# rmcolq/charon

Measured on AMD Instinct MI355X. Metric: classified reads/sec + achieved HBM GB/s vs roofline, 5 kb reads, 39 GB index, higher is better.
Workload: dtype u64

## Files before the change

charon_amd/csrc/charon_hip.hip:

```cpp

#include <hip/hip_runtime.h>

#include <algorithm>
#include <chrono>
#include <functional>
#include <cmath>
#include <cstddef>
#include <cstdint>
#include <cstdio>
#include <cstdlib>
#include <cstring>
#include <limits>
#include <mutex>
#include <new>
#include <string>
#include <type_traits>
#include <vector>

#include "charon_hip.h"
#include "default_kde.inc"

#include "parts/common.inc"
#include "parts/lds_budget.hpp"
#include "parts/k1_minimise_probe.inc"
#include "parts/k2_count_wavelog.inc"
#include "parts/shard_kernels.inc"
#include "parts/shardx_kernels.inc"
#include "parts/k3_model_call.inc"
#include "parts/len_order.inc"
#include "parts/gzip_trees.inc"
#include "parts/gzip_walk.inc"
#include "parts/gzip_tally.inc"
#include "parts/gzip_size_dev.inc"
#include "parts/gzip_tally_long.inc"
#include "parts/text_pack.inc"
#include "parts/text_split.inc"
#include "parts/fasta_split.inc"
#include "parts/text_gather.inc"
#include "parts/text_pair.inc"
#include "parts/extract_records.inc"
#include "parts/inflate_members.inc"
#include "parts/deflate_members.inc"
#include "parts/ef_decode.inc"
#include "parts/synth_kernels.inc"
#include "parts/abi_index_model.inc"
#include "parts/abi_stream_batch.inc"
#include "parts/abi_shard_wait.inc"
#include "parts/abi_text_split.inc"
#include "parts/abi_fasta_split.inc"
#include "parts/abi_text_fetch.inc"
#include "parts/abi_text_pair.inc"
#include "parts/abi_text_batch.inc"
#include "parts/abi_inflate.inc"
#include "parts/abi_deflate.inc"
#include "parts/abi_extract.inc"
#include "parts/abi_shardx.inc"
#include "parts/abi_synth_memory.inc"
```

charon_amd/csrc/parts/abi_shard_wait.inc:

```

static int ensure_shard_buffers(chn_stream *s) {
    const uint64_t nw = (s->cfg.max_reads + WAVE - 1) / WAVE;
    int rc;
    if ((rc = s->big.ensure(s->cfg.max_bases, nw, (uint32_t)s->idx->d.bin_words, 65536, 0))) return rc;
    if ((rc = s->d_list.ensure(s->big.log_cap * 8)) || (rc = s->d_cbase.ensure((nw + 1) * 8))) return rc;
    return CHN_OK;
}
static ShardArgs shard_args(chn_stream *s, const chn_index *shard, uint64_t *partial, const Slot &sl) {
    ShardArgs a;
    std::memset(&a, 0, sizeof a);
    const chn_index_desc &d = shard->d;
    a.list = s->d_list.as<uint64_t>(); a.wave_meta = s->big.meta.as<WaveMeta>(); a.cbase = s->d_cbase.as<uint64_t>();
    a.wave_count = s->big.wcount.as<uint32_t>(); a.words = shard->words; a.S = d.bin_size; a.row_begin = d.row_begin; a.row_end = d.row_end;
    a.shift = (uint32_t)d.hash_shift; a.h = d.hash_funs; a.W = (uint32_t)d.bin_words; a.partial = partial; a.rows = s->big.rows.as<uint64_t>();
    a.rowlog = s->big.log.as<uint32_t>(); a.B = (uint32_t)d.bins;
    a.n_waves = (uint32_t)((sl.n_reads + WAVE - 1) / WAVE); a.esc_capacity = s->big.esc_cap;
    a.status = reinterpret_cast<uint32_t *>(const_cast<Slot &>(sl).d_ctl.as<unsigned long long>() + CTL_STATUS);
    return a;
}

extern "C" int chn_shard_minimise(chn_stream *s, const chn_batch *b, uint64_t *n_entries) {
    if (!s || !b || !n_entries) return fail(CHN_E_INVALID, "chn_shard_minimise: null argument");
    if (s->shard_open || s->shx_stage != 0) return fail(CHN_E_STATE, "chn_shard_minimise: previous sharded batch not finished");
    HIPCHK(hipSetDevice(s->idx->d.device));
// ... 84 lines not shown
    HIPCHK(hipStreamSynchronize(s->stream));
    return CHN_OK;
}

extern "C" int chn_shard_finish(chn_stream *s, const uint64_t *dev_partial) {
    if (!s) return fail(CHN_E_INVALID, "chn_shard_finish: null argument");
    if (!s->shard_open) return fail(CHN_E_STATE, "chn_shard_finish: no sharded batch open");
    if (!dev_partial && s->shard_entries) return fail(CHN_E_INVALID, "chn_shard_finish: null argument");
    HIPCHK(hipSetDevice(s->idx->d.device));
    Slot &sl = s->slot[s->head];
    const uint32_t n_waves = (uint32_t)((sl.n_reads + WAVE - 1) / WAVE);
    const ShardArgs sa = shard_args(s, s->idx, const_cast<uint64_t *>(dev_partial), sl);
    switch (s->idx->d.bin_words) {
        case 1: hipLaunchKernelGGL(k_and_partial<1>, dim3(n_waves), dim3(256), 0, s->stream, sa); break;
        case 2: hipLaunchKernelGGL(k_and_partial<2>, dim3(n_waves), dim3(256), 0, s->stream, sa); break;
        case 3: hipLaunchKernelGGL(k_and_partial<3>, dim3(n_waves), dim3(256), 0, s->stream, sa); break;
        default: hipLaunchKernelGGL(k_and_partial<4>, dim3(n_waves), dim3(256), 0, s->stream, sa); break;
    }
    HIPCHK(hipGetLastError());
    s->shard_open = false;
    HIPCHK(hipEventRecord(sl.k1_done, s->stream));
    HIPCHK(hipStreamWaitEvent(s->stream2, sl.k1_done, 0));
    int rc = launch_tail(s, sl, s->big, s->stream2);
    if (rc) return rc;
    s->head = (s->head + 1) % chn_stream::N_SLOTS;
    s->inflight += 1;
    return CHN_OK;
}

extern "C" int chn_stream_sync(chn_stream *s) {
    if (!s) return fail(CHN_E_INVALID, "null stream");
    HIPCHK(hipSetDevice(s->idx->d.device));
    HIPCHK(hipStreamSynchronize(s->stream0));
    HIPCHK(hipStreamSynchronize(s->stream));
    HIPCHK(hipStreamSynchronize(s->stream1));
    HIPCHK(hipStreamSynchronize(s->stream4));
    HIPCHK(hipStreamSynchronize(s->stream2));
    return CHN_OK;
}

static int rerun_worst_case(chn_stream *s, Slot &sl) {
    const chn_index_desc &d = s->idx->d;
    unsigned long long *ctl = sl.d_ctl.as<unsigned long long>();
    const uint64_t n = sl.n_reads, nw = (n + WAVE - 1) / WAVE + sl.split_bound;
    HIPCHK(hipMemsetAsync(ctl, 0, CTL_NLONG * 8, s->stream));
    HIPCHK(hipMemsetAsync(ctl + CTL_FETCHES, 0, (CTL_WORDS - CTL_FETCHES) * 8, s->stream));
    hipLaunchKernelGGL(k_sum_len, dim3((uint32_t)std::min<uint64_t>(1024, (n + 255) / 256)), dim3(256), 0, s->stream, sl.len1, sl.len2, (uint32_t)n, ctl + CTL_WORDS - 1);
    HIPCHK(hipGetLastError());
    unsigned long long total = 0;
    HIPCHK(hipMemcpyAsync(&total, ctl + CTL_WORDS - 1, 8, hipMemcpyDeviceToHost, s->stream));
    HIPCHK(hipStreamSynchronize(s->stream));
    int rc = s->big.ensure(total, (n + WAVE - 1) / WAVE + std::min<uint64_t>(sl.split_bound, total / len_bucket_floor(std::min(s->long_bucket, 247u)) + 1), (uint32_t)d.bin_words, 65536, 0, nw);
    if (rc) return rc;
    K1Args a = sl.k1;
    a.gate_started = a.gate_signal = nullptr;
    fill_k1_log(a, sl, s->big, true);
    const size_t lds = k1_lds_bytes(a.wn, d.num_categories, MODE_ROWS, a.h, (uint32_t)d.bin_words, (uint32_t)d.bins, a.pack != 0);
    hipError_t e = launch_k1_mode(MODE_ROWS, (uint32_t)d.bin_words, a, lds, s->stream);
    if (e == hipSuccess && sl.split_bound) e = launch_k1_split_mode(MODE_ROWS, (uint32_t)d.bin_words, a, lds, s->stream, split_grid(sl.split_bound));
    if (e != hipSuccess) return fail(CHN_E_HIP, std::string("k_minimise_probe re-run: ") + hipGetErrorString(e));
    if ((rc = launch_tail(s, sl, s->big, s->stream))) return rc;
    HIPCHK(hipStreamSynchronize(s->stream));
    s->overflow_reruns += 1;
    return CHN_OK;
}

extern "C" int chn_batch_wait(chn_stream *s, chn_result *r) {
    if (!s || !r || r->struct_size != sizeof(chn_result)) return fail(CHN_E_INVALID, "chn_batch_wait: bad argument");
    if (s->inflight == 0) return fail(CHN_E_STATE, "no batch in flight");
    HIPCHK(hipSetDevice(s->idx->d.device));
    Slot &sl = s->slot[(s->head + chn_stream::N_SLOTS - s->inflight) % chn_stream::N_SLOTS];
    static const bool diag_wait = diag_env("CHN_DIAG_WAIT") != nullptr;
    auto dnow = []() { return std::chrono::duration<double>(std::chrono::steady_clock::now().time_since_epoch()).count(); };
    const double dw0 = diag_wait ? dnow() : 0;
    HIPCHK(hipEventSynchronize(sl.done));
    const double dw1 = diag_wait ? dnow() : 0;
    if (sl.want_gzt) HIPCHK(hipEventSynchronize(sl.gz_done));
    const double dw2 = diag_wait ? dnow() : 0;
    struct DiagPrint { bool on; double a, b, c; std::function<double()> now; ~DiagPrint() { if (on) std::fprintf(stderr, "chn_batch_wait: at %.4f  done-event %.2f ms  gz-event %.2f ms  rest %.2f ms\n", a, (b - a) * 1e3, (c - b) * 1e3, (now() - c) * 1e3); } } diag_print{diag_wait, dw0, dw1, dw2, dnow};
    s->inflight -= 1;
    static const int evpair[4][2] = {{0, 1}, {2, 3}, {4, 5}, {6, 7}};
    for (int i = 0; i < 4; ++i)
        if (sl.ev_used[i]) {
            float ms = 0;
            HIPCHK(hipEventElapsedTime(&ms, sl.ev[evpair[i][0]], sl.ev[evpair[i][1]]));
            if (i == 0) {
                float t0 = 0, t1 = 0;
                HIPCHK(hipEventElapsedTime(&t0, s->prof_anchor[s->prof_cur], sl.ev[0]));
                HIPCHK(hipEventElapsedTime(&t1, s->prof_anchor[s->prof_cur], sl.ev[1]));
                if (s->prof_have_end && s->prof_prev_end > (double)t0) ms = (float)std::max(0.0, (double)t1 - s->prof_prev_end);
                if (!s->prof_have_end || (double)t1 > s->prof_prev_end) s->prof_prev_end = t1;
                s->prof_have_end = true;
                if (sl.new_anchor) {
                    float off = 0;
                    HIPCHK(hipEventElapsedTime(&off, s->prof_anchor[s->prof_cur], s->prof_anchor[s->prof_cur ^ 1]));
                    s->prof_prev_end -= off; s->prof_cur ^= 1;
                    sl.new_anchor = s->prof_anchor_pending = false;
                }
            }
            s->prof_ms[i] += ms; s->prof_n[i] += 1;
        }
    unsigned long long ctl[CTL_WORDS];
    const uint64_t n = sl.n_reads, C = s->idx->d.num_categories;
    const ResLayout L(n, C);
    const char *staged = sl.staged ? sl.h_res.as<char>() : nullptr;
    if (staged) std::memcpy(ctl, staged + L.ctl, sizeof ctl);
// ... 193 lines not shown
```

charon_amd/csrc/parts/abi_stream_batch.inc:

```

struct ResLayout {
    size_t ctl, prob, nh, counts, unique, call, conf, flags, total;
    ResLayout(uint64_t n, uint64_t C) {
        ctl = 0; prob = CTL_WORDS * 8; nh = prob + n * C * 8; counts = nh + n * 4; unique = counts + n * C * 4; call = unique + n * C * 4;
        conf = call + n; flags = conf + n; total = flags + n;
    }
};

static const int PROF_ANCHOR_SECONDS = 8;
static hipError_t prof_anchor_now(chn_stream *s) {
    for (Slot &sl : s->slot) sl.new_anchor = false;
    s->prof_cur = 0; s->prof_anchor_pending = false; s->prof_have_end = false; s->prof_prev_end = 0;
    hipError_t e = hipEventRecord(s->prof_anchor[0], s->stream);
    if (e == hipSuccess) e = hipEventSynchronize(s->prof_anchor[0]);
    s->prof_anchor_at = std::chrono::steady_clock::now();
    return e;
}

extern "C" int chn_stream_create(chn_index *idx, const chn_stream_cfg *cfg, chn_stream **out) {
    if (!idx || !cfg || !out || cfg->struct_size != sizeof(chn_stream_cfg)) return fail(CHN_E_INVALID, "chn_stream_create: bad argument");
    if (cfg->max_reads == 0 || cfg->max_reads > 0xFFFFFF00ULL) return fail(CHN_E_INVALID, "max_reads out of range");
    HIPCHK(hipSetDevice(idx->d.device));
    idx->ef_release();
    chn_stream *s = new (std::nothrow) chn_stream();
// ... 516 lines not shown
    HIPCHK(hipGetLastError());
    HIPCHK(hipEventRecord(sl.uploaded, s->stream0));
    HIPCHK(hipStreamWaitEvent(ps, sl.uploaded, 0));

    K1Args &a = sl.k1;
    std::memset(&a, 0, sizeof(a));
    a.words = s->idx->words; a.S = d.bin_size; a.row_begin = d.row_begin; a.row_end = d.row_end; a.seed = d.minimiser_seed; a.powk1 = pow5(d.kmer_size - 1);
    a.shift = (uint32_t)d.hash_shift; a.h = d.hash_funs; a.k = d.kmer_size; a.wn = d.window_size - d.kmer_size + 1;
    a.n_reads = (uint32_t)n; a.nseg = paired ? 2 : 1; a.B = (uint32_t)d.bins; a.C = C;
    a.pack = ring_pack_ok(a.k, a.wn, a.seed) ? 1u : 0u;
    for (uint32_t bb = 0; bb < 8 && bb < d.bins; ++bb) a.b2c_packed |= (uint64_t)d.bin_to_category[bb] << (8 * bb);
    a.bases = bases; a.nmask = nmask; a.off1 = off1; a.off2 = off2; a.len1 = sl.len1; a.len2 = sl.len2; a.n_bases = b->n_bases;
    a.order = sl.d_order.as<uint32_t>();
    a.status = reinterpret_cast<uint32_t *>(ctl + CTL_STATUS);
    if (const char *ab = diag_env("CHN_ABLATE")) a.ablate = (uint32_t)std::atoi(ab);
    a.nt_probes = s->idx->rows_local * d.bin_words * 8 > (4ULL << 30) ? 1u : 0u;
    if (const char *nt = diag_env("CHN_NT_PROBES")) a.nt_probes = (uint32_t)std::atoi(nt);
    a.num_hashes = sl.d_num_hashes.as<uint32_t>(); a.counts = sl.d_counts.as<uint32_t>(); a.unique = sl.d_unique.as<uint32_t>();
    const uint32_t n_waves = (uint32_t)((n + WAVE - 1) / WAVE);
    a.n_long_ptr = sl.split_bound ? ctl + CTL_NLONG : nullptr; a.wave_slot0 = n_waves;
    a.fetches = ctl + CTL_FETCHES;
    if (list_kind == LIST_SPARSE) {
        fill_k1_log(a, sl, s->shx, true);
        a.rows = s->d_list.as<uint64_t>();
    } else if (list_mode) {
        fill_k1_log(a, sl, s->big, false);
        a.rows = s->d_list.as<uint64_t>();
        hipLaunchKernelGGL(k_wave_caps, dim3((uint32_t)((n + 255) / 256)), dim3(256), 0, ps, sl.d_order.as<uint32_t>(), sl.len1, sl.len2,
                           (uint32_t)n, s->big.cap_num, s->big.esc_shift, s->big.meta.as<WaveMeta>());
        hipLaunchKernelGGL(k_scan_meta, dim3(1), dim3(1024), 0, ps, s->big.meta.as<WaveMeta>(), n_waves);
        HIPCHK(hipGetLastError());
    } else if (!fused) {
        fill_k1_log(a, sl, sl.lb, true);
    }
    const int mode = list_mode ? MODE_LIST : fused ? MODE_FUSED : MODE_ROWS;
    size_t lds = k1_lds_bytes(a.wn, C, mode, a.h, W, a.B, a.pack != 0);
    if (const char *pad = diag_env("CHN_LDS_PAD")) lds += (size_t)std::atoi(pad);
    if (lds > 160 * 1024) return fail(CHN_E_INVALID, "window too large for LDS");
    if (sl.split_bound) {
        HIPCHK(hipStreamWaitEvent(s->stream4, sl.uploaded, 0));
        hipError_t e4 = launch_k1_split_mode(mode, W, a, lds, s->stream4, split_grid(sl.split_bound));
        if (e4 != hipSuccess) return fail(CHN_E_HIP, std::string("k_minimise_probe (split) launch: ") + hipGetErrorString(e4));
        HIPCHK(hipEventRecord(sl.split_done, s->stream4));
    }
    const bool gated = !list_mode && alternate && s->gate_signal != nullptr;
    if (gated) {
        if (s->gate_seq) {
            HIPCHK(hipStreamWaitValue64(ps, s->gate_signal, s->gate_seq, hipStreamWaitValueGte, ~0ull));
            s->gated_batches += 1;
        }
        a.gate_started = ctl + CTL_GATE; a.gate_signal = s->gate_signal; a.gate_value = s->gate_seq + 1;
    }
    if (prof) { HIPCHK(hipEventRecord(sl.ev[0], ps)); }
    hipError_t e = launch_k1_mode(mode, W, a, lds, ps);
    if (e != hipSuccess) return fail(CHN_E_HIP, std::string("k_minimise_probe launch: ") + hipGetErrorString(e));
    if (gated) s->gate_seq += 1;
    if (prof) {
        if (sl.split_bound) HIPCHK(hipStreamWaitEvent(ps, sl.split_done, 0));
        HIPCHK(hipEventRecord(sl.ev[1], ps)); sl.ev_used[0] = true;
        if (!s->prof_anchor_pending && std::chrono::steady_clock::now() - s->prof_anchor_at > std::chrono::seconds(PROF_ANCHOR_SECONDS)) {
            HIPCHK(hipEventRecord(s->prof_anchor[s->prof_cur ^ 1], ps));
            s->prof_anchor_at = std::chrono::steady_clock::now();
            sl.new_anchor = s->prof_anchor_pending = true;
        }
    }

    if (list_mode) return CHN_OK;
    dt[3] = dnow();
    HIPCHK(hipEventRecord(sl.k1_done, ps));
    HIPCHK(hipStreamWaitEvent(s->stream2, sl.k1_done, 0));
    if (sl.split_bound) HIPCHK(hipStreamWaitEvent(s->stream2, sl.split_done, 0));
    if (gated) {
        hipLaunchKernelGGL(k_gate_release, dim3(1), dim3(1), 0, ps, s->gate_signal, (unsigned long long)s->gate_seq);
        HIPCHK(hipGetLastError());
    }
    int rc = launch_tail(s, sl, sl.lb, s->stream2);
    if (rc) return rc;
    if (diag_sub) std::fprintf(stderr, "submit: validate + uploads %.2f ms, deflate tallies %.2f, ordering + probe launch %.2f, tail %.2f\n",
                               (dt[1] - dt[0]) * 1e3, (dt[2] - dt[1]) * 1e3, (dt[3] - dt[2]) * 1e3, (dnow() - dt[3]) * 1e3);
    s->head = (s->head + 1) % chn_stream::N_SLOTS;
    s->inflight += 1;
    s->batch_seq += 1;
    return CHN_OK;
}


static int launch_tail(chn_stream *s, Slot &sl, LogBuf &lb, hipStream_t st) {
    const chn_index_desc &d = s->idx->d;
    const uint64_t n = sl.n_reads;
    const uint32_t W = (uint32_t)d.bin_words, C = d.num_categories;
    const uint32_t n_waves = (uint32_t)((n + WAVE - 1) / WAVE);
    const bool prof = (s->cfg.flags & CHN_STREAM_PROFILE) != 0 && st == s->stream2;
    unsigned long long *ctl = sl.d_ctl.as<unsigned long long>();
    if (!sl.fused) {
        K2Args k2;
        std::memset(&k2, 0, sizeof(k2));
        k2.rows = lb.rows.as<uint64_t>(); k2.rowlog = lb.log.as<uint32_t>();
        k2.wave_meta = lb.meta.as<WaveMeta>(); k2.wave_count = lb.wcount.as<uint32_t>(); k2.order = sl.d_order.as<uint32_t>();
        k2.counts = sl.d_counts.as<uint32_t>(); k2.unique = sl.d_unique.as<uint32_t>();
        k2.n_reads = (uint32_t)n; k2.B = (uint32_t)d.bins; k2.C = C; k2.W = W;
        std::memcpy(k2.b2c, d.bin_to_category, 256);
        k2.n_long_ptr = sl.split_bound && !sl.list_mode ? ctl + CTL_NLONG : nullptr; k2.wave_slot0 = n_waves;
        const dim3 grid(n_waves), block(K2_THREADS);
        const bool t16 = !sl.list_mode && sl.len2 == nullptr && s->long_bucket <= LONG_BUCKET_DEFAULT;
        const uint32_t wn = d.window_size - d.kmer_size + 1;
        const size_t probe_lds = k1_lds_bytes(wn, C, MODE_ROWS, d.hash_funs, W, (uint32_t)d.bins, ring_pack_ok(d.kmer_size, wn, d.minimiser_seed));
        const uint32_t G = k2_group((uint32_t)d.bins, C, W, t16, k2_lds_budget(probe_lds));
        k2.group = G;
        const size_t lds2 = k2_lds_bytes((uint32_t)d.bins, C, W, G, t16);
        if (lds2 > 150 * 1024) return fail(CHN_E_INVALID, "bins x categories too large for the count kernel's LDS");
        const void *fn = t16 ? (W == 1 ? (const void *)k_count_wavelog<1, true> : W == 2 ? (const void *)k_count_wavelog<2, true> : W == 3 ? (const void *)k_count_wavelog<3, true> : (const void *)k_count_wavelog<4, true>)
                             : (W == 1 ? (const void *)k_count_wavelog<1, false> : W == 2 ? (const void *)k_count_wavelog<2, false> : W == 3 ? (const void *)k_count_wavelog<3, false> : (const void *)k_count_wavelog<4, false>);
        if (lds2 > 48 * 1024) HIPCHK(hipFuncSetAttribute(fn, hipFuncAttributeMaxDynamicSharedMemorySize, (int)lds2));
        if (prof) HIPCHK(hipEventRecord(sl.ev[2], st));
        {
            void *args[] = {(void *)&k2};
            HIPCHK(hipLaunchKernel(fn, grid, block, args, lds2, st));
        }
        if (k2.n_long_ptr) {
            const dim3 lgrid(std::min<uint32_t>(sl.split_bound, 4096u)), lblock(K2L_THREADS);
            switch (W) {
                case 1: hipLaunchKernelGGL(k_count_longlog<1>, lgrid, lblock, 0, st, k2); break;
                case 2: hipLaunchKernelGGL(k_count_longlog<2>, lgrid, lblock, 0, st, k2); break;
                case 3: hipLaunchKernelGGL(k_count_longlog<3>, lgrid, lblock, 0, st, k2); break;
                default: hipLaunchKernelGGL(k_count_longlog<4>, lgrid, lblock, 0, st, k2); break;
            }
        }
        HIPCHK(hipGetLastError());
        if (prof) { HIPCHK(hipEventRecord(sl.ev[3], st)); sl.ev_used[1] = true; }
    }
    sl.model_ran = s->model.set;
    const uint32_t hW8 = (uint32_t)(d.hash_funs * W * 8), outb = (uint32_t)(8 + 8 * C);
    if (s->model.set) {
        K3Args k3 = s->k3;
        k3.num_hashes = sl.d_num_hashes.as<uint32_t>(); k3.counts = sl.d_counts.as<uint32_t>(); k3.unique = sl.d_unique.as<uint32_t>();
        k3.len1 = sl.len1; k3.len2 = sl.len2; k3.mean_quality = sl.mq; k3.compression = sl.comp;
        k3.prob = sl.d_prob.as<double>(); k3.call = sl.d_call.as<uint8_t>(); k3.conf = sl.d_conf.as<uint8_t>(); k3.flags = sl.d_flags.as<uint8_t>();
        k3.n_reads = (uint32_t)n;
        k3.acc = ctl + CTL_BYTES; k3.hW8 = hW8; k3.outb = outb;
        k3.open_compression_gate = sl.want_gzt ? 1u : 0u;
        if (prof) HIPCHK(hipEventRecord(sl.ev[4], st));
        hipLaunchKernelGGL(k_model_call, dim3((uint32_t)((n + 255) / 256)), dim3(256), 0, st, k3);
        HIPCHK(hipGetLastError());
        if (prof) { HIPCHK(hipEventRecord(sl.ev[5], st)); sl.ev_used[2] = true; }
    } else {
        hipLaunchKernelGGL(k_batch_bytes, dim3((uint32_t)std::min<uint64_t>(1024, (n + 255) / 256)), dim3(256), 0, st, sl.len1, sl.len2,
                           sl.d_num_hashes.as<uint32_t>(), (uint32_t)n, hW8, outb, ctl + CTL_BYTES);
        HIPCHK(hipGetLastError());
    }
    if (prof) { HIPCHK(hipEventRecord(sl.ev[7], st)); sl.ev_used[3] = true; }
    sl.staged = false;
    if (st == s->stream2 && sl.host_batch) {
        const ResLayout L(n, C);
        int rc = sl.h_res.ensure(L.total);
        if (rc) return rc;
// ... 27 lines not shown
```

charon_amd/csrc/parts/k1_minimise_probe.inc:

```

#ifndef CHN_LOG_BATCH
#define CHN_LOG_BATCH 4
#endif
#ifndef CHN_BASE_PIECES
#define CHN_BASE_PIECES 4
#endif

#ifndef K1_COND_MAX_BINS
#define K1_COND_MAX_BINS 4u
#endif
#ifndef FUSED_ROUNDS
#define FUSED_ROUNDS 2u
#endif

struct WaveMeta { uint64_t base, esc_base; uint32_t cap, esc_cap, pad0, pad1; };

struct K1Args {
    const uint64_t *words;
    uint64_t *words_rw;
    uint64_t S, row_begin, row_end, seed, powk1;
    uint32_t shift, h, k, wn, n_reads, nseg, B, C;
    uint64_t b2c_packed;
    const uint32_t *bases, *nmask;
    const uint64_t *off1, *off2;
    const uint32_t *len1, *len2;
    const uint32_t *order;
    uint32_t *num_hashes, *counts, *unique;
    uint64_t *rows;
    uint32_t *rowlog;
    WaveMeta *wave_meta;
    uint32_t *wave_count;
    unsigned long long *cursor;
    uint64_t log_capacity, esc_capacity;
    uint32_t cap_num, esc_shift;
    uint32_t *status;
    uint64_t n_bases;
    uint32_t nt_probes;
    const uint8_t *read_bin;
    uint32_t ablate;
    uint32_t pack;
    const unsigned long long *n_long_ptr;
    uint32_t wave_slot0;
    unsigned long long *fetches;
    unsigned long long *gate_started, *gate_signal;
    unsigned long long gate_value;
};
__global__ void k_gate_release(unsigned long long *signal, unsigned long long value) {
    if (threadIdx.x == 0 && blockIdx.x == 0) [[clang::atomic(remote_memory, fine_grained_memory)]] {
        (void)__hip_atomic_fetch_max(signal, value, __ATOMIC_RELAXED, __HIP_MEMORY_SCOPE_SYSTEM);
    }
}

__device__ bool first_window_tied(const K1Args &a, uint64_t o, uint32_t wn) {
    const uint64_t INV5 = 0xCCCCCCCCCCCCCCCDULL;
    const uint32_t k = a.k, w = wn + k - 1;
    uint64_t fwd = 0, rc = 0, best = ~0ULL;
    bool tie = false;
    auto digits = [&](uint64_t x, uint32_t &d, uint32_t &cd) {
        const uint32_t code = (a.bases[x >> 4] >> ((x & 15u) * 2u)) & 3u;
        const uint32_t nf = a.nmask ? (a.nmask[x >> 5] >> (x & 31u)) & 1u : 0u;
        d = nf ? 3u : code + (code == 3u);
        cd = nf ? 3u : (3u - code) + (code == 0u);
    };
    for (uint32_t i = 0; i < w; ++i) {
        uint32_t d_in, cd_in, d_out = 0, cd_out = 0;
        digits(o + i, d_in, cd_in);
        if (i >= k) digits(o + i - k, d_out, cd_out);
        fwd = (fwd - (uint64_t)d_out * a.powk1) * 5u + d_in;
        rc = (rc - cd_out) * INV5 + (uint64_t)cd_in * a.powk1;
        if (i + 1 >= k) {
            const uint64_t vf = fwd ^ a.seed, vr = rc ^ a.seed, v = vf < vr ? vf : vr;
            if (v < best) { best = v; tie = false; } else if (v == best) tie = true;
        }
    }
    return tie;
}

#define ROWLOG_ESC_MASK 0x03fffffcu
#define ROWLOG_ESC_MAX 0x00fffffeu
__host__ __device__ __forceinline__ uint64_t wave_log_cap(uint64_t sum_len, uint32_t cap_num) { return (((sum_len * cap_num) >> 16) + 64 + 63) & ~63ULL; }
__host__ __device__ __forceinline__ uint64_t wave_esc_cap(uint64_t cap, uint32_t esc_shift) { return (cap >> esc_shift) + 64; }
template <int W>
__device__ __forceinline__ uint32_t encode_row(const uint64_t *acc, uint32_t B, uint32_t owner, bool &escaped) {
    uint64_t m[W];
    uint32_t pc = 0;
#pragma unroll
    for (int w = 0; w < W; ++w) {
        m[w] = acc[w];
        if (w == W - 1 && (B & 63u)) m[w] &= (1ULL << (B & 63u)) - 1;
        pc += (uint32_t)__popcll(m[w]);
    }
    escaped = pc > 3;
    if (escaped) return owner << 26;
    uint32_t e = pc | (owner << 26), slot = 0;
#pragma unroll
    for (int w = 0; w < W; ++w) {
        uint64_t x = m[w];
        while (x) {
            const uint32_t b = (uint32_t)w * 64 + (uint32_t)__ffsll((long long)x) - 1;
            x &= x - 1;
            e |= b << (2 + 8 * slot);
            ++slot;
        }
    }
    return e;
}

__device__ __forceinline__ void lds_dma_b128(const void *src, uint32_t lds_dst, bool nt) {
    unsigned keep;
    const uint32_t dst = (uint32_t)__builtin_amdgcn_readfirstlane((int)lds_dst);
    if (nt)
        asm volatile("s_mov_b32 %0, m0\n\ts_mov_b32 m0, %2\n\ts_nop 0\n\tglobal_load_lds_dwordx4 %1, off nt\n\ts_mov_b32 m0, %0"
                     : "=&s"(keep) : "v"(src), "s"(dst) : "memory");
    else
        asm volatile("s_mov_b32 %0, m0\n\ts_mov_b32 m0, %2\n\ts_nop 0\n\tglobal_load_lds_dwordx4 %1, off\n\ts_mov_b32 m0, %0"
                     : "=&s"(keep) : "v"(src), "s"(dst) : "memory");
}
__device__ __forceinline__ void wait_vmcnt(uint32_t n) {
    switch (n) {
        case 0: asm volatile("s_waitcnt vmcnt(0)" ::: "memory"); break;
        case 1: asm volatile("s_waitcnt vmcnt(1)" ::: "memory"); break;
        case 2: asm volatile("s_waitcnt vmcnt(2)" ::: "memory"); break;
        case 3: asm volatile("s_waitcnt vmcnt(3)" ::: "memory"); break;
        case 4: asm volatile("s_waitcnt vmcnt(4)" ::: "memory"); break;
        case 5: asm volatile("s_waitcnt vmcnt(5)" ::: "memory"); break;
        case 6: asm volatile("s_waitcnt vmcnt(6)" ::: "memory"); break;
        case 7: asm volatile("s_waitcnt vmcnt(6)" ::: "memory"); break;
        case 8: asm volatile("s_waitcnt vmcnt(8)" ::: "memory"); break;
        case 9: asm volatile("s_waitcnt vmcnt(8)" ::: "memory"); break;
        default: asm volatile("s_waitcnt vmcnt(10)" ::: "memory"); break;
    }
}

__host__ __device__ constexpr uint32_t ring_pbits(uint32_t wn) {
    uint32_t n = 0;
    for (uint32_t x = wn - 1; x; x >>= 1) ++n;
    return n;
}
template <int W, int MODE, int WN_T, bool SPLIT = false, bool COND_T = false>
__global__ __launch_bounds__(WAVE) void k_minimise_probe(const K1Args a) {
    extern __shared__ __align__(16) unsigned char smem[];
    if (!SPLIT && a.gate_started && threadIdx.x == 0) {
        if (atomicAdd(a.gate_started, 1ULL) == (unsigned long long)gridDim.x - 1) [[clang::atomic(remote_memory, fine_grained_memory)]] {
            (void)__hip_atomic_fetch_max(a.gate_signal, a.gate_value, __ATOMIC_RELAXED, __HIP_MEMORY_SCOPE_SYSTEM);
        }
    }
    const uint32_t n_long = a.n_long_ptr ? (uint32_t)__builtin_nontemporal_load(a.n_long_ptr) : 0u;
    uint32_t item = blockIdx.x;
    if (SPLIT && item >= n_long) return;
    do {
    const uint32_t wslot = SPLIT ? a.wave_slot0 + item : item;
    const uint32_t wn = WN_T ? (uint32_t)WN_T : a.wn;
    constexpr uint32_t NBLK = (W == 1 || W == 2) ? 1u : 2u;
    constexpr bool COND = MODE == MODE_FUSED && COND_T;
    constexpr uint32_t QC = COND ? QCAP + WAVE : QCAP;
    auto qwrap = [&](uint32_t x) -> uint32_t {
        if (!COND) return x & (QC - 1);
        x = x >= QC ? x - QC : x;
// ... 61 lines not shown
    }
    uint32_t read_len = seg_len0;
    if (SPLIT) {
        const uint32_t w = wn + a.k - 1, Lr = seg_len0;
        const uint64_t roff = seg_off0;
        const uint32_t P = Lr > w + 64u ? min(64u, (Lr - w) >> 6) : 1u;
        const uint32_t start = lane < P ? (uint32_t)(((uint64_t)lane * (Lr - w)) / P) & ~63u : 0u;
        const bool tied = lane > 0 && lane < P && first_window_tied(a, roff + start, wn);
        const uint64_t alive = __ballot(lane < P && !tied) | 1ULL;
        seg_len0 = 0;
        if ((alive >> lane) & 1ULL) {
            const uint64_t above = lane == 63 ? 0ULL : alive >> (lane + 1);
            uint32_t end = Lr;
            if (above) {
                const uint32_t nx = lane + 1 + (uint32_t)__ffsll((long long)above) - 1;
                end = ((uint32_t)(((uint64_t)nx * (Lr - w)) / P) & ~63u) + w;
            }
            seg_off0 = roff + start; seg_len0 = end - start; cold = lane > 0;
        }
    }
    uint64_t wbase = 0, ebase = 0;
    uint32_t wcap = 0, ecap = 0;
    if (MODE == MODE_ROWS || MODE == MODE_LIST) {
        if (a.cursor) {
            uint64_t sum = (uint64_t)seg_len0 + seg_len1;
            for (int o = 32; o > 0; o >>= 1) sum += (uint64_t)__shfl_xor((long long)sum, o);
            if (SPLIT) sum = read_len;
            const uint64_t cap = wave_log_cap(sum, a.cap_num), ec = wave_esc_cap(cap, a.esc_shift);
            uint64_t b0 = 0, b1 = 0;
            if (lane == 0) {
                b0 = atomicAdd(a.cursor, (unsigned long long)cap);
                b1 = atomicAdd(a.cursor + 1, (unsigned long long)ec);
                a.wave_meta[wslot].base = b0;
                a.wave_meta[wslot].esc_base = b1;
            }
            wbase = (uint64_t)__shfl((long long)b0, 0);
            ebase = (uint64_t)__shfl((long long)b1, 0);
            const uint64_t room = wbase < a.log_capacity ? a.log_capacity - wbase : 0, eroom = ebase < a.esc_capacity ? a.esc_capacity - ebase : 0;
            wcap = (uint32_t)(cap < room ? cap : room);
            ecap = (uint32_t)(ec < eroom ? ec : eroom);
            if (wcap > 0xffffffc0u) wcap = 0xffffffc0u;
        } else {
            wbase = a.wave_meta[wslot].base; ebase = a.wave_meta[wslot].esc_base;
            const uint64_t wend = wslot + 1 < gridDim.x ? a.wave_meta[wslot + 1].base : a.log_capacity;
            const uint64_t eend = wslot + 1 < gridDim.x ? a.wave_meta[wslot + 1].esc_base : a.esc_capacity;
            const uint64_t c = (wend < a.log_capacity ? wend : a.log_capacity), ce = (eend < a.esc_capacity ? eend : a.esc_capacity);
            wcap = (uint32_t)(c > wbase ? (c - wbase < 0xffffffc0ULL ? c - wbase : 0xffffffc0ULL) : 0);
            ecap = (uint32_t)(ce > ebase ? (ce - ebase < 0xffffffc0ULL ? ce - ebase : 0xffffffc0ULL) : 0);
        }
        if (ecap > ROWLOG_ESC_MAX) ecap = ROWLOG_ESC_MAX;
        if (lane == 0) { a.wave_meta[wslot].cap = wcap; a.wave_meta[wslot].esc_cap = ecap; }
    }
    bool overflow = false;
    uint32_t staged = 0, flushed = 0;

    auto log_flush = [&](uint32_t first, uint32_t count) {
        asm volatile("s_waitcnt lgkmcnt(0)" ::: "memory");
#pragma unroll
        for (uint32_t t4 = 0; t4 < CHN_LOG_BATCH * WAVE / 4; t4 += WAVE) {
            const uint32_t q4 = t4 + lane;
            if (q4 * 4 < count) {
                const uint4 v = reinterpret_cast<const uint4 *>(sbuf)[q4];
                *reinterpret_cast<uint4 *>(a.rowlog + wbase + first + q4 * 4) = v;
            }
        }
    };

    auto probe_retire = [&]() {
        const uint32_t slot = r_retired & 1u;
        const uint32_t newer = r_issued - r_retired - 1u;
        wait_vmcnt((a.ablate & 3u) ? 0u : newer * a.h * NBLK);
        if (newer == 0u || base_seq < r_issued) base_ready = true;
        const uint32_t n = slot ? n_s1 : n_s0, meta = slot ? meta_s1 : meta_s0, sel = slot ? sel_s1 : sel_s0;
        const bool has = lane < n;
        uint64_t acc[W];
#pragma unroll
        for (int w = 0; w < W; ++w) acc[w] = ~0ULL;
        const uint4 *pb4 = reinterpret_cast<const uint4 *>(pbuf + slot * pb_round);
#pragma unroll
        for (uint32_t i = 0; i < 5; ++i)
            if (i < a.h) {
                const uint4 v0 = pb4[(i * NBLK) * WAVE + lane];
                const uint64_t q0 = (uint64_t)v0.x | ((uint64_t)v0.y << 32), q1 = (uint64_t)v0.z | ((uint64_t)v0.w << 32);
                if (W == 1) {
                    acc[0] &= ((sel >> i) & 1u) ? q1 : q0;
                } else if (W == 2) {
                    acc[0] &= q0; acc[W > 1 ? 1 : 0] &= q1;
                } else {
                    const uint4 v1 = pb4[(i * NBLK + (NBLK - 1)) * WAVE + lane];
                    const uint64_t q2 = (uint64_t)v1.x | ((uint64_t)v1.y << 32), q3 = (uint64_t)v1.z | ((uint64_t)v1.w << 32);
                    if (W == 3) {
                        const bool odd = (sel >> i) & 1u;
                        acc[0] &= odd ? q1 : q0; acc[W > 1 ? 1 : 0] &= odd ? q2 : q1; acc[W > 2 ? 2 : 0] &= odd ? q3 : q2;
                    } else {
                        acc[0] &= q0; acc[W > 1 ? 1 : 0] &= q1; acc[W > 2 ? 2 : 0] &= q2; acc[W > 3 ? 3 : 0] &= q3;
                    }
                }
            }
        const uint32_t owner = meta & 63u;
        if (MODE == MODE_FUSED) {
            uint64_t m = has ? (acc[0] & ((a.B >= 64) ? ~0ULL : ((1ULL << a.B) - 1))) : 0;
            const bool single = __popcll(m) == 1;
            while (m) {
                const uint32_t b = (uint32_t)__ffsll((long long)m) - 1;
                m &= m - 1;
                const uint32_t c = (uint32_t)(a.b2c_packed >> (8 * b)) & 0xffu;
                atomicAdd(&cnt[c * WAVE + owner], 1u);
                if (single) atomicAdd(&unq[c * WAVE + owner], 1u);
            }
        } else if (MODE == MODE_ROWS) {
            bool esc = false;
            uint32_t entry = 0;
            if (has) entry = encode_row<W>(acc, a.B, owner, esc);
            const bool keep = has && (esc || (entry & 0x03ffffffu) != 0);
            const uint64_t km = __ballot(keep);
            const uint32_t nk = (uint32_t)__popcll(km);
            const uint32_t krank = __builtin_amdgcn_mbcnt_hi((uint32_t)(km >> 32), __builtin_amdgcn_mbcnt_lo((uint32_t)km, 0u));
            const bool fits = consumed + nk <= wcap;
            const uint64_t em = __ballot(esc);
            if (em) {
                const uint32_t ne = (uint32_t)__popcll(em);
                const uint32_t eslot = esc_n + __builtin_amdgcn_mbcnt_hi((uint32_t)(em >> 32), __builtin_amdgcn_mbcnt_lo((uint32_t)em, 0u));
                if (esc_n + ne > ecap) overflow = true;
                else if (esc && fits) {
#ifndef CHN_DIAG_NO_ESC_STORE
                    uint64_t *dst = a.rows + (ebase + eslot) * W;
#pragma unroll
                    for (int w = 0; w < W; ++w) dst[w] = acc[w];
#endif
                    entry |= (eslot + 1) << 2;
                }
                esc_n += ne;
            }
#ifndef CHN_DIAG_NO_STORE
            if (CHN_LOG_BATCH == 1) {
                if (keep && fits) a.rowlog[wbase + consumed + krank] = entry;
            } else {
                if (keep) sbuf[staged + krank] = entry;
                staged += nk;
                if (staged >= CHN_LOG_BATCH * WAVE) {
                    if (fits) log_flush(flushed, CHN_LOG_BATCH * WAVE);
                    flushed += CHN_LOG_BATCH * WAVE;
                    const uint32_t rem = staged - CHN_LOG_BATCH * WAVE;
                    uint32_t t = 0;
                    if (lane < rem) t = sbuf[CHN_LOG_BATCH * WAVE + lane];
                    asm volatile("s_waitcnt lgkmcnt(0)" ::: "memory");
                    if (lane < rem) sbuf[lane] = t;
                    staged = rem;
                }
            }
#endif
            if (!fits) overflow = true;
            consumed += nk;
        }
        r_retired += 1;
    };

    auto probe_issue = [&](uint32_t n_take) {
        asm volatile("s_waitcnt lgkmcnt(0)" ::: "memory");
        const bool has = lane < n_take;
        const uint32_t qslot = qwrap(qhead + lane);
        const uint64_t val = qv[qslot];
        const uint32_t meta = qm[qslot];
        const uint32_t slot = r_issued & 1u;
        uint32_t sel = 0;
        if (has) {
            const uint32_t dst_lds = pbuf_lds + slot * pb_round;
#pragma unroll
            for (uint32_t i = 0; i < 5; ++i)
                if (i < a.h) {
                    const uint64_t row = hash_and_fit_row(val, c_ibf_seeds[i], a.S, a.shift);
                    const uint64_t o = (row - a.row_begin) * (8u * W);
                    if (W & 1) sel |= (uint32_t)((o >> 3) & 1u) << i;
                    const unsigned char *src = reinterpret_cast<const unsigned char *>(a.words) + (o & ~15ULL);
                    if (a.ablate & 3u) continue;
#pragma unroll
                    for (uint32_t j = 0; j < NBLK; ++j) lds_dma_b128(src + 16 * j, dst_lds + (i * NBLK + j) * 1024u, a.nt_probes != 0);
                }
        }
        if (slot) { meta_s1 = meta; sel_s1 = sel; n_s1 = n_take; } else { meta_s0 = meta; sel_s0 = sel; n_s0 = n_take; }
        n_fetch += n_take * a.h;
        r_issued += 1;
        qhead = qwrap(qhead + n_take);
        qcount -= n_take;
    };

    uint64_t fv[FUSED_ROUNDS], fa[FUSED_ROUNDS];
    uint32_t fm[FUSED_ROUNDS], fn[FUSED_ROUNDS];
#pragma unroll
    for (uint32_t sidx = 0; sidx < FUSED_ROUNDS; ++sidx) { fv[sidx] = 0; fa[sidx] = 0; fm[sidx] = 0; fn[sidx] = 0; }
    const uint64_t binmask = (a.B >= 64) ? ~0ULL : ((1ULL << a.B) - 1);
// ... 395 lines not shown
```

charon_amd/csrc/parts/k2_count_wavelog.inc:

```

struct K2Args {
    const uint64_t *rows;
    const uint32_t *rowlog;
    const WaveMeta *wave_meta;
    const uint32_t *wave_count;
    const uint32_t *order;
    uint32_t *counts, *unique;
    uint32_t n_reads, B, C, W;
    uint8_t b2c[256];
    const unsigned long long *n_long_ptr;
    uint32_t wave_slot0;
    uint32_t group;
};

#define K2_THREADS 512
#define K2_UNROLL 4
template <int W, bool T16>
__global__ __launch_bounds__(K2_THREADS) void k_count_wavelog(const K2Args a) {
    extern __shared__ __align__(16) unsigned char smem2[];
    __builtin_amdgcn_s_setprio(3);
    const uint32_t B = a.B, C = a.C, G = a.group;
    const uint32_t TB = T16 ? (B + 1) / 2 : B;
    uint32_t *tot = reinterpret_cast<uint32_t *>(smem2);
    uint32_t *unq = tot + (size_t)G * TB;
    uint64_t *cmask = reinterpret_cast<uint64_t *>(unq + (size_t)G * C + ((G * C) & 1u));
    uint8_t *chosen = reinterpret_cast<uint8_t *>(cmask + G * W);
    __shared__ uint8_t s_b2c[256];
    const uint32_t tid = threadIdx.x, g = blockIdx.x;
    const uint32_t n_long = a.n_long_ptr ? (uint32_t)*a.n_long_ptr : 0u;
    if ((g + 1) * WAVE <= n_long) return;
    if (tid < 256) s_b2c[tid] = a.b2c[tid];
    const uint32_t count = a.wave_count[g];
    const uint64_t *rows = a.rows + a.wave_meta[g].esc_base * W;
    const uint32_t *log = a.rowlog + a.wave_meta[g].base;
    const uint64_t lastmask = (B & 63u) ? ((1ULL << (B & 63u)) - 1) : ~0ULL;
    const uint4 *log4 = reinterpret_cast<const uint4 *>(log);
    const uint32_t count4 = (count + 3) / 4;
    auto bump = [&](uint32_t o, uint32_t b) {
        if (T16) atomicAdd(&tot[o * TB + (b >> 1)], 1u << (16u * (b & 1u)));
        else atomicAdd(&tot[o * TB + b], 1u);
    };
    auto total = [&](uint32_t o, uint32_t b) -> uint32_t { return T16 ? (tot[o * TB + (b >> 1)] >> (16u * (b & 1u))) & 0xffffu : tot[o * TB + b]; };
    auto sweep = [&](auto f) {
        for (uint32_t i4 = tid; i4 < count4; i4 += K2_THREADS * K2_UNROLL) {
            uint4 v[K2_UNROLL];
#pragma unroll
            for (int u = 0; u < K2_UNROLL; ++u) {
                const uint32_t j = i4 + u * K2_THREADS;
                v[u] = j < count4 ? log4[j] : make_uint4(0, 0, 0, 0);
            }
#pragma unroll
            for (int u = 0; u < K2_UNROLL; ++u) {
                const uint32_t xs[4] = {v[u].x, v[u].y, v[u].z, v[u].w};
#pragma unroll
                for (int q = 0; q < 4; ++q)
                    if ((i4 + u * K2_THREADS) * 4 + q < count) f(xs[q]);
            }
        }
    };
    for (uint32_t o0 = 0; o0 < WAVE; o0 += G) {
        __syncthreads();
        for (uint32_t i = tid; i < G * TB; i += K2_THREADS) tot[i] = 0;
        for (uint32_t i = tid; i < G * C; i += K2_THREADS) { unq[i] = 0; chosen[i] = 255; }
        for (uint32_t i = tid; i < G * W; i += K2_THREADS) cmask[i] = 0;
        __syncthreads();
        sweep([&](uint32_t x) {
            const uint32_t o = (x >> 26) - o0, pc = x & 3u;
            if (o >= G) return;
            if (pc) {
                bump(o, (x >> 2) & 0xffu);
                if (pc > 1) bump(o, (x >> 10) & 0xffu);
                if (pc > 2) bump(o, (x >> 18) & 0xffu);
            } else if (x & ROWLOG_ESC_MASK) {
                const size_t j = ((x & ROWLOG_ESC_MASK) >> 2) - 1;
#pragma unroll
                for (int w = 0; w < W; ++w) {
                    uint64_t r = rows[j * W + w];
                    if (w == W - 1) r &= lastmask;
                    while (r) {
                        const uint32_t b = (uint32_t)__ffsll((long long)r) - 1;
                        r &= r - 1;
                        bump(o, w * 64 + b);
                    }
                }
            }
        });
        __syncthreads();
        for (uint32_t i = tid; i < G * C; i += K2_THREADS) {
            const uint32_t o = i / C, c = i % C;
            uint32_t best = 255, bestv = 0;
            for (uint32_t b = 0; b < B; ++b) {
                const uint32_t t = total(o, b);
                if (s_b2c[b] == c && (best == 255 || t > bestv)) { best = b; bestv = t; }
            }
            chosen[i] = (uint8_t)best;
            if (best != 255) atomicOr((unsigned long long *)&cmask[o * W + (best >> 6)], 1ULL << (best & 63u));
            const uint32_t gi = g * WAVE + o0 + o;
            if (gi < a.n_reads && gi >= n_long) a.counts[(size_t)a.order[gi] * C + c] = best == 255 ? 0u : bestv;
        }
        __syncthreads();
        sweep([&](uint32_t x) {
            const uint32_t o = (x >> 26) - o0, pc = x & 3u;
            if (o >= G) return;
            uint32_t found = 0, fbin = 0;
            if (pc) {
                for (uint32_t j = 0; j < pc; ++j) {
                    const uint32_t b = (x >> (2 + 8 * j)) & 0xffu;
                    if ((cmask[o * W + (b >> 6)] >> (b & 63u)) & 1ULL) { ++found; fbin = b; }
                }
            } else if (x & ROWLOG_ESC_MASK) {
                const size_t j = ((x & ROWLOG_ESC_MASK) >> 2) - 1;
#pragma unroll
                for (int w = 0; w < W; ++w) {
                    const uint64_t r = rows[j * W + w] & cmask[o * W + w];
                    found += (uint32_t)__popcll(r);
                    if (r) fbin = w * 64 + (uint32_t)__ffsll((long long)r) - 1;
                }
            }
            if (found == 1) atomicAdd(&unq[o * C + s_b2c[fbin]], 1u);
        });
        __syncthreads();
        for (uint32_t i = tid; i < G * C; i += K2_THREADS) {
            const uint32_t o = i / C, c = i % C, gi = g * WAVE + o0 + o;
            if (gi < a.n_reads && gi >= n_long) a.unique[(size_t)a.order[gi] * C + c] = unq[i];
        }
    }
}
#define K2L_THREADS 256
template <int W>
__global__ __launch_bounds__(K2L_THREADS) void k_count_longlog(const K2Args a) {
    __shared__ uint32_t tot[256], unq[256];
    __shared__ uint64_t cmask[4];
    __shared__ uint8_t s_b2c[256];
    const uint32_t B = a.B, C = a.C, tid = threadIdx.x;
    const uint32_t n_long = a.n_long_ptr ? (uint32_t)*a.n_long_ptr : 0u;
    s_b2c[tid] = a.b2c[tid];
    const uint64_t lastmask = (B & 63u) ? ((1ULL << (B & 63u)) - 1) : ~0ULL;
    for (uint32_t item = blockIdx.x; item < n_long; item += gridDim.x) {
        const uint32_t g = a.wave_slot0 + item, r = a.order[item];
        __syncthreads();
        tot[tid] = 0; unq[tid] = 0;
        if (tid < 4) cmask[tid] = 0;
        __syncthreads();
        const uint32_t count = a.wave_count[g];
        const uint64_t *rows = a.rows + a.wave_meta[g].esc_base * W;
        const uint32_t *log = a.rowlog + a.wave_meta[g].base;
        for (uint32_t e = tid; e < count; e += K2L_THREADS) {
            const uint32_t x = log[e], pc = x & 3u;
            if (pc) {
                atomicAdd(&tot[(x >> 2) & 0xffu], 1u);
                if (pc > 1) atomicAdd(&tot[(x >> 10) & 0xffu], 1u);
                if (pc > 2) atomicAdd(&tot[(x >> 18) & 0xffu], 1u);
            } else if (x & ROWLOG_ESC_MASK) {
                const size_t j = ((x & ROWLOG_ESC_MASK) >> 2) - 1;
#pragma unroll
                for (int w = 0; w < W; ++w) {
                    uint64_t rw = rows[j * W + w];
                    if (w == W - 1) rw &= lastmask;
                    while (rw) { const uint32_t b = (uint32_t)__ffsll((long long)rw) - 1; rw &= rw - 1; atomicAdd(&tot[w * 64 + b], 1u); }
                }
            }
        }
// ... 72 lines not shown
```

Measured before the change: 35.45 million.

## Chain two rowlog entries to encode up to six bins before escaping

Result: faster. 36.07 million, median of 6 (+1.7%).

```diff
diff --git a/charon_amd/csrc/charon_hip.hip b/charon_amd/csrc/charon_hip.hip
--- a/charon_amd/csrc/charon_hip.hip
+++ b/charon_amd/csrc/charon_hip.hip
@@ -22,6 +22,7 @@
 
 #include "parts/common.inc"
 #include "parts/lds_budget.hpp"
+#include "parts/rowlog_entry.hpp"
 #include "parts/k1_minimise_probe.inc"
 #include "parts/k2_count_wavelog.inc"
 #include "parts/shard_kernels.inc"
diff --git a/charon_amd/csrc/parts/abi_shard_wait.inc b/charon_amd/csrc/parts/abi_shard_wait.inc
--- a/charon_amd/csrc/parts/abi_shard_wait.inc
+++ b/charon_amd/csrc/parts/abi_shard_wait.inc
@@ -160,6 +160,7 @@
     HIPCHK(hipStreamSynchronize(s->stream));
     int rc = s->big.ensure(total, (n + WAVE - 1) / WAVE + std::min<uint64_t>(sl.split_bound, total / len_bucket_floor(std::min(s->long_bucket, 247u)) + 1), (uint32_t)d.bin_words, 65536, 0, nw);
     if (rc) return rc;
+    sl.k1.chain = 0;
     K1Args a = sl.k1;
     a.gate_started = a.gate_signal = nullptr;
     fill_k1_log(a, sl, s->big, true);
diff --git a/charon_amd/csrc/parts/abi_stream_batch.inc b/charon_amd/csrc/parts/abi_stream_batch.inc
--- a/charon_amd/csrc/parts/abi_stream_batch.inc
+++ b/charon_amd/csrc/parts/abi_stream_batch.inc
@@ -592,6 +592,7 @@
         a.gate_started = ctl + CTL_GATE; a.gate_signal = s->gate_signal; a.gate_value = s->gate_seq + 1;
     }
     if (prof) { HIPCHK(hipEventRecord(sl.ev[0], ps)); }
+    a.chain = (mode == MODE_ROWS && rowlog_chain_ok(a.B)) ? 1u : 0u;
     hipError_t e = launch_k1_mode(mode, W, a, lds, ps);
     if (e != hipSuccess) return fail(CHN_E_HIP, std::string("k_minimise_probe launch: ") + hipGetErrorString(e));
     if (gated) s->gate_seq += 1;
@@ -641,6 +642,7 @@
         k2.n_reads = (uint32_t)n; k2.B = (uint32_t)d.bins; k2.C = C; k2.W = W;
         std::memcpy(k2.b2c, d.bin_to_category, 256);
         k2.n_long_ptr = sl.split_bound && !sl.list_mode ? ctl + CTL_NLONG : nullptr; k2.wave_slot0 = n_waves;
+        k2.chain = sl.list_mode ? 0u : sl.k1.chain;
         const dim3 grid(n_waves), block(K2_THREADS);
         const bool t16 = !sl.list_mode && sl.len2 == nullptr && s->long_bucket <= LONG_BUCKET_DEFAULT;
         const uint32_t wn = d.window_size - d.kmer_size + 1;
diff --git a/charon_amd/csrc/parts/k1_minimise_probe.inc b/charon_amd/csrc/parts/k1_minimise_probe.inc
--- a/charon_amd/csrc/parts/k1_minimise_probe.inc
+++ b/charon_amd/csrc/parts/k1_minimise_probe.inc
@@ -39,6 +39,7 @@
     const uint8_t *read_bin;
     uint32_t ablate;
     uint32_t pack;
+    uint32_t chain;
     const unsigned long long *n_long_ptr;
     uint32_t wave_slot0;
     unsigned long long *fetches;
@@ -76,34 +77,13 @@
     return tie;
 }
 
-#define ROWLOG_ESC_MASK 0x03fffffcu
-#define ROWLOG_ESC_MAX 0x00fffffeu
 __host__ __device__ __forceinline__ uint64_t wave_log_cap(uint64_t sum_len, uint32_t cap_num) { return (((sum_len * cap_num) >> 16) + 64 + 63) & ~63ULL; }
 __host__ __device__ __forceinline__ uint64_t wave_esc_cap(uint64_t cap, uint32_t esc_shift) { return (cap >> esc_shift) + 64; }
 template <int W>
 __device__ __forceinline__ uint32_t encode_row(const uint64_t *acc, uint32_t B, uint32_t owner, bool &escaped) {
-    uint64_t m[W];
-    uint32_t pc = 0;
-#pragma unroll
-    for (int w = 0; w < W; ++w) {
-        m[w] = acc[w];
-        if (w == W - 1 && (B & 63u)) m[w] &= (1ULL << (B & 63u)) - 1;
-        pc += (uint32_t)__popcll(m[w]);
-    }
-    escaped = pc > 3;
-    if (escaped) return owner << 26;
-    uint32_t e = pc | (owner << 26), slot = 0;
-#pragma unroll
-    for (int w = 0; w < W; ++w) {
-        uint64_t x = m[w];
-        while (x) {
-            const uint32_t b = (uint32_t)w * 64 + (uint32_t)__ffsll((long long)x) - 1;
-            x &= x - 1;
-            e |= b << (2 + 8 * slot);
-            ++slot;
-        }
-    }
-    return e;
+    uint32_t e[2];
+    rowlog_encode<W>(acc, B, owner, false, e, escaped);
+    return e[0];
 }
 
 __device__ __forceinline__ void lds_dma_b128(const void *src, uint32_t lds_dst, bool nt) {
@@ -271,6 +251,7 @@
         if (lane == 0) { a.wave_meta[wslot].cap = wcap; a.wave_meta[wslot].esc_cap = ecap; }
     }
     bool overflow = false;
+    const bool chain = MODE == MODE_ROWS && !SPLIT && a.chain != 0;
     uint32_t staged = 0, flushed = 0;
 
     auto log_flush = [&](uint32_t first, uint32_t count) {
@@ -329,12 +310,14 @@
             }
         } else if (MODE == MODE_ROWS) {
             bool esc = false;
-            uint32_t entry = 0;
-            if (has) entry = encode_row<W>(acc, a.B, owner, esc);
-            const bool keep = has && (esc || (entry & 0x03ffffffu) != 0);
-            const uint64_t km = __ballot(keep);
-            const uint32_t nk = (uint32_t)__popcll(km);
-            const uint32_t krank = __builtin_amdgcn_mbcnt_hi((uint32_t)(km >> 32), __builtin_amdgcn_mbcnt_lo((uint32_t)km, 0u));
+            uint32_t ent[2] = {0u, 0u}, ne = 0;
+            if (has) ne = rowlog_encode<W>(acc, a.B, owner, chain, ent, esc);
+            uint32_t entry = ent[0];
+            const bool keep = ne != 0, two = ne == 2;
+            const uint64_t km = __ballot(keep), tm = __ballot(two);
+            const uint32_t nk = (uint32_t)__popcll(km) + (uint32_t)__popcll(tm);
+            const uint32_t krank = __builtin_amdgcn_mbcnt_hi((uint32_t)(km >> 32), __builtin_amdgcn_mbcnt_lo((uint32_t)km, 0u)) +
+                                   __builtin_amdgcn_mbcnt_hi((uint32_t)(tm >> 32), __builtin_amdgcn_mbcnt_lo((uint32_t)tm, 0u));
             const bool fits = consumed + nk <= wcap;
             const uint64_t em = __ballot(esc);
             if (em) {
@@ -354,8 +337,21 @@
 #ifndef CHN_DIAG_NO_STORE
             if (CHN_LOG_BATCH == 1) {
                 if (keep && fits) a.rowlog[wbase + consumed + krank] = entry;
+                if (two && fits) a.rowlog[wbase + consumed + krank + 1] = ent[1];
             } else {
+                if (staged + nk > (CHN_LOG_BATCH + 1) * WAVE) {
+                    const uint32_t whole = staged & ~(WAVE - 1u);
+                    if (fits) log_flush(flushed, whole);
+                    flushed += whole;
+                    const uint32_t rem = staged - whole;
+                    uint32_t t = 0;
+                    if (lane < rem) t = sbuf[whole + lane];
+                    asm volatile("s_waitcnt lgkmcnt(0)" ::: "memory");
+                    if (lane < rem) sbuf[lane] = t;
+                    staged = rem;
+                }
                 if (keep) sbuf[staged + krank] = entry;
+                if (two) sbuf[staged + krank + 1] = ent[1];
                 staged += nk;
                 if (staged >= CHN_LOG_BATCH * WAVE) {
                     if (fits) log_flush(flushed, CHN_LOG_BATCH * WAVE);
diff --git a/charon_amd/csrc/parts/k2_count_wavelog.inc b/charon_amd/csrc/parts/k2_count_wavelog.inc
--- a/charon_amd/csrc/parts/k2_count_wavelog.inc
+++ b/charon_amd/csrc/parts/k2_count_wavelog.inc
@@ -11,6 +11,7 @@
     const unsigned long long *n_long_ptr;
     uint32_t wave_slot0;
     uint32_t group;
+    uint32_t chain;
 };
 
 #define K2_THREADS 512
@@ -20,6 +21,7 @@
     extern __shared__ __align__(16) unsigned char smem2[];
     __builtin_amdgcn_s_setprio(3);
     const uint32_t B = a.B, C = a.C, G = a.group;
+    const bool chain = a.chain != 0;
     const uint32_t TB = T16 ? (B + 1) / 2 : B;
     uint32_t *tot = reinterpret_cast<uint32_t *>(smem2);
     uint32_t *unq = tot + (size_t)G * TB;
@@ -54,7 +56,7 @@
                 const uint32_t xs[4] = {v[u].x, v[u].y, v[u].z, v[u].w};
 #pragma unroll
                 for (int q = 0; q < 4; ++q)
-                    if ((i4 + u * K2_THREADS) * 4 + q < count) f(xs[q]);
+                    if ((i4 + u * K2_THREADS) * 4 + q < count) f(xs[q], (i4 + u * K2_THREADS) * 4 + q);
             }
         }
     };
@@ -64,13 +66,13 @@
         for (uint32_t i = tid; i < G * C; i += K2_THREADS) { unq[i] = 0; chosen[i] = 255; }
         for (uint32_t i = tid; i < G * W; i += K2_THREADS) cmask[i] = 0;
         __syncthreads();
-        sweep([&](uint32_t x) {
-            const uint32_t o = (x >> 26) - o0, pc = x & 3u;
+        sweep([&](uint32_t x, uint32_t) {
+            const uint32_t o = (x >> 26) - o0, pc = rowlog_count(x);
             if (o >= G) return;
             if (pc) {
-                bump(o, (x >> 2) & 0xffu);
-                if (pc > 1) bump(o, (x >> 10) & 0xffu);
-                if (pc > 2) bump(o, (x >> 18) & 0xffu);
+                bump(o, rowlog_bin(x, 0, chain));
+                if (pc > 1) bump(o, rowlog_bin(x, 1, chain));
+                if (pc > 2) bump(o, rowlog_bin(x, 2, chain));
             } else if (x & ROWLOG_ESC_MASK) {
                 const size_t j = ((x & ROWLOG_ESC_MASK) >> 2) - 1;
 #pragma unroll
@@ -99,15 +101,15 @@
             if (gi < a.n_reads && gi >= n_long) a.counts[(size_t)a.order[gi] * C + c] = best == 255 ? 0u : bestv;
         }
         __syncthreads();
-        sweep([&](uint32_t x) {
-            const uint32_t o = (x >> 26) - o0, pc = x & 3u;
+        sweep([&](uint32_t x, uint32_t e) {
+            const uint32_t o = (x >> 26) - o0, pc = rowlog_count(x);
             if (o >= G) return;
             uint32_t found = 0, fbin = 0;
             if (pc) {
-                for (uint32_t j = 0; j < pc; ++j) {
-                    const uint32_t b = (x >> (2 + 8 * j)) & 0xffu;
-                    if ((cmask[o * W + (b >> 6)] >> (b & 63u)) & 1ULL) { ++found; fbin = b; }
-                }
+                if (rowlog_is_tail(x, chain)) return;
+                auto is_chosen = [&](uint32_t b) -> bool { return (cmask[o * W + (b >> 6)] >> (b & 63u)) & 1ULL; };
+                found = rowlog_match(x, chain, is_chosen, fbin);
+                if (rowlog_has_tail(x, chain)) found += rowlog_match(rowlog_tail(log, e, count, chain), chain, is_chosen, fbin);
             } else if (x & ROWLOG_ESC_MASK) {
                 const size_t j = ((x & ROWLOG_ESC_MASK) >> 2) - 1;
 #pragma unroll
diff --git a/charon_amd/csrc/parts/rowlog_entry.hpp b/charon_amd/csrc/parts/rowlog_entry.hpp
--- /dev/null
+++ b/charon_amd/csrc/parts/rowlog_entry.hpp
@@ -0,0 +1,71 @@
+#ifndef CHN_ROWLOG_ENTRY_HPP
+#define CHN_ROWLOG_ENTRY_HPP
+
+#include <cstdint>
+
+#if defined(__HIPCC__) || defined(__CUDACC__)
+#define ROWLOG_HD __host__ __device__ __forceinline__
+#else
+#define ROWLOG_HD static inline
+#endif
+
+#define ROWLOG_ESC_MASK 0x03fffffcu
+#define ROWLOG_ESC_MAX 0x00fffffeu
+#define ROWLOG_CHAIN_NEXT (1u << 9)
+#define ROWLOG_CHAIN_PREV (1u << 17)
+#define ROWLOG_CHAIN_MAX_BINS 128u
+
+ROWLOG_HD bool rowlog_chain_ok(uint32_t B) { return B <= ROWLOG_CHAIN_MAX_BINS; }
+ROWLOG_HD uint32_t rowlog_bin_mask(bool chain) { return chain ? 0x7fu : 0xffu; }
+
+template <int W>
+ROWLOG_HD uint32_t rowlog_encode(const uint64_t *acc, uint32_t B, uint32_t owner, bool chain, uint32_t e[2], bool &escaped) {
+    uint64_t m[W];
+    uint32_t pc = 0;
+    for (int w = 0; w < W; ++w) {
+        m[w] = acc[w];
+        if (w == W - 1 && (B & 63u)) m[w] &= (1ULL << (B & 63u)) - 1;
+        pc += (uint32_t)__builtin_popcountll(m[w]);
+    }
+    e[0] = e[1] = owner << 26;
+    escaped = pc > (chain ? 6u : 3u);
+    if (escaped) return 1;
+    if (pc == 0) return 0;
+    const uint32_t n = pc > 3 ? 2u : 1u;
+    e[0] |= pc > 3 ? 3u | ROWLOG_CHAIN_NEXT : pc;
+    if (n == 2) e[1] |= (pc - 3) | ROWLOG_CHAIN_PREV;
+    uint32_t slot = 0;
+    for (int w = 0; w < W; ++w) {
+        uint64_t x = m[w];
+        while (x) {
+            const uint32_t b = (uint32_t)w * 64 + (uint32_t)__builtin_ctzll(x);
+            x &= x - 1;
+            if (slot < 3) e[0] |= b << (2 + 8 * slot); else e[1] |= b << (2 + 8 * (slot - 3));
+            ++slot;
+        }
+    }
+    return n;
+}
+
+ROWLOG_HD uint32_t rowlog_count(uint32_t x) { return x & 3u; }
+ROWLOG_HD uint32_t rowlog_bin(uint32_t x, uint32_t j, bool chain) { return (x >> (2 + 8 * j)) & rowlog_bin_mask(chain); }
+ROWLOG_HD bool rowlog_is_tail(uint32_t x, bool chain) { return chain && (x & 3u) != 0 && (x & ROWLOG_CHAIN_PREV) != 0; }
+ROWLOG_HD bool rowlog_has_tail(uint32_t x, bool chain) { return chain && (x & 3u) != 0 && (x & ROWLOG_CHAIN_NEXT) != 0; }
+template <class Log>
+ROWLOG_HD uint32_t rowlog_tail(const Log &log, uint32_t e, uint32_t count, bool chain) {
+    if (e + 1 >= count) return 0;
+    const uint32_t y = log[e + 1];
+    return rowlog_is_tail(y, chain) ? y : 0u;
+}
+template <class Chosen>
+ROWLOG_HD uint32_t rowlog_match(uint32_t x, bool chain, const Chosen &chosen, uint32_t &fbin) {
+    uint32_t found = 0;
+    const uint32_t pc = rowlog_count(x);
+    for (uint32_t j = 0; j < pc; ++j) {
+        const uint32_t b = rowlog_bin(x, j, chain);
+        if (chosen(b)) { ++found; fbin = b; }
+    }
+    return found;
+}
+
+#endif
```
